# gregversteeg/LinearCorex

Hardware: NVIDIA B200
Metric: fit_iters_per_sec (higher is better)
Workload: dtype f64 (6 int8 digit planes = 48 bits, exact int32 products, f64 recombination)

## Files before the change

### linearcorex_b200/csrc/host_gram.cuh

```cuda
#pragma once
#include "host_oz.cuh"

static long long gram_tbuf_doubles(const lcx_session* s, int block_cols) {
    return ((long long)s->L.S * block_cols * s->L.ldk8 + 7) / 8;
}

static long long gram_scratch_doubles(const lcx_session* s, int block_cols, long long ldg) {
    return round_up(block_cols, 16) + align16(gram_tbuf_doubles(s, block_cols)) +
           (s->L.oz_build_splits > 1 ? (long long)s->L.oz_build_splits * block_cols * ldg : 0LL) + 64;
}

template <int S>
static int gram_build_t(lcx_session* s, double* g, long long ldg, int B, double* scratch) {
    const Layout& L = s->L;
    const int n = s->n;
    double* scale = scratch;
    int8_t* tbuf = (int8_t*)(scratch + round_up(B, 16));
    double* part = scratch + round_up(B, 16) + align16(gram_tbuf_doubles(s, B));
    const long long t_stride = (long long)B * L.ldk8;
    const int splits = L.oz_build_splits;
    oz::gram_scale_kernel<<<cdiv(B, 256), 256, 0, s->stream>>>(s->oz_xscale(), 1.0 / (double)s->Nt, scale, B);
    LAUNCHED(s);
    for (int c0 = 0; c0 < n; c0 += B) {
        const int nb = min(B, n - c0);
        oz::transpose_planes_kernel<<<dim3((unsigned)cdiv(s->Nl, 128), cdiv(nb, 128), S), dim3(32, 8), 0, s->stream>>>(
            s->xs(), L.ld8, s->Nl, s->Nl * L.ld8, c0, nb, tbuf, L.ldk8, t_stride);
        LAUNCHED(s);
        const int bnm = oz::bn_max(S);
        const int n_tiles = cdiv(nb, bnm);
        const int bn = (int)max(16LL, round_up(cdiv(nb, n_tiles), bnm > 64 ? 16 : 8));
        CUtensorMap map_a, map_b;
        LCX_TRY(oz::make_slice_map(&map_a, s->xs() + c0, n - c0, s->Nl, S, L.ld8, s->Nl * L.ld8, oz::kBM, oz::kBK, true));
        LCX_TRY(oz::make_slice_map(&map_b, tbuf, s->Nl, nb, S, L.ldk8, t_stride, oz::kBK, bn, false));
        oz::GemmParams p;
        memset(&p, 0, sizeof(p));
        double* dst = g + (long long)c0 * ldg + c0;
        p.C = splits > 1 ? part : dst;
        p.ldc = ldg;
        p.c_split_stride = splits > 1 ? (long long)B * ldg : 0;
        p.col_scale = scale;
        p.inv_radix = 1.0 / (double)L.radix;
        p.rows = n - c0; p.cols = nb; p.k_total = (int)s->Nl; p.k_chunk = L.oz_build_chunk;
        p.bn = bn;
        p.trans_out = 1;
        LCX_TRY((oz::launch_oz_gemm<S, false>(map_a, map_b, p, dim3(n_tiles, cdiv(n - c0, oz::kBM), splits), s->stream, oz_cluster())));
        LAUNCHED(s);
        if (splits > 1) {
            LCX_TRY(launch_reduce_splits(part, splits, (long long)B * ldg, dst, nb, n - c0, ldg, s->stream));
            LAUNCHED(s);
        }
    }
    oz::mirror_upper_kernel<<<dim3(cdiv(n, 32), cdiv(n, 32)), dim3(32, 8), 0, s->stream>>>(g, ldg, n);
    LAUNCHED(s);
    LCX_CUDA(cudaGetLastError());
    return 0;
}

static int gram_build(lcx_session* s, double* g, long long ldg, int B, double* scratch) {
    switch (s->L.S) {
        case 3: return gram_build_t<3>(s, g, ldg, B, scratch);
        case 4: return gram_build_t<4>(s, g, ldg, B, scratch);
        case 5: return gram_build_t<5>(s, g, ldg, B, scratch);
        case 6: return gram_build_t<6>(s, g, ldg, B, scratch);
        case 7: return gram_build_t<7>(s, g, ldg, B, scratch);
    }
    return fail(LCX_ERR_STATE, "gram_build", "bad digit count");
}

template <int S>
static int gram_pair_t(lcx_session* s, const double* A, double* svec, cudaEvent_t* ev, const double* dot_b, double* dot_out,
                       bool leave_partials) {
    const Layout& L = s->L;
    const int m = s->m, n = s->n;
    double* D = s->ptr(LCX_A_D);
    if (s->row_parts > 0 && dot_out != nullptr) {
        oz::slice_rows_part_kernel<S><<<dim3(m, cdiv(L.ld8, 4 * 128)), 128, 0, s->stream>>>(
            A, L.ld, m, n, s->ptr(I_FROW), s->ptr(I_FROW) + (long long)kSMs * L.ldm, s->row_parts, L.ldm, s->oz_xscale(),
            s->oz_ascale(), s->oz_cscale(), dot_out, s->as(), L.ld8, (long long)m * L.ld8, (double)L.radix);
        LAUNCHED(s);
    } else {
    oz::row_scale_kernel<<<m, 256, 0, s->stream>>>(A, L.ld, n, s->oz_ascale(), 0, s->oz_xscale(), s->oz_cscale(), dot_b, dot_out);
    LAUNCHED(s);
    oz::slice_rows_kernel<S><<<dim3(m, cdiv(L.ld8, 4 * 128)), 128, 0, s->stream>>>(A, L.ld, m, n, s->oz_ascale(), nullptr, s->as(), L.ld8,
                                                                              (long long)m * L.ld8, (double)L.radix);
    LAUNCHED(s);
    }
    oz::GemmParams p;
    memset(&p, 0, sizeof(p));
    p.ldc = L.ld;
    p.col_scale = s->oz_cscale();
    p.inv_radix = 1.0 / (double)L.radix;
    p.rows = n; p.cols = m; p.k_total = n;
    p.bn = s->oz_bn;
    p.trans_out = 1;
    s->d_splits = 1;
    const int n_tiles = cdiv(m, oz::bn_max(S));
    if (s->peers.world > 1) {
        const int P = s->peers.world, m_tiles = cdiv(n, oz::kBM);
        const int per = cdiv(m_tiles, P);
        const int t0 = min(m_tiles, s->peers.rank * per), t1 = min(m_tiles, t0 + per);
        const int mine = t1 - t0;
        const int clusters = kSMs / 2, kblocks = cdiv(n, oz::kBK);
        const long long col0 = (long long)t0 * oz::kBM;
        const int ncols = (int)(min((long long)L.ld, (long long)t1 * oz::kBM) - col0);
        if (mine > 0) {
            const int smin = cdiv(n, L.oz_kmax), smax = max(smin, min(clusters, max(1, kblocks / 4)));
            int sp = smin;
            double best = 1e300;
            for (int c = smin; c <= smax; ++c) {
                const int rounds = cdiv((long long)mine * c, clusters);
                const double cost = rounds * (ceil((double)kblocks / c) + oz_unit_fixed_kb()) + (c > 1 ? 1.5 * c : 0.0);
                if (cost < best - 1e-9) { best = cost; sp = c; }
            }
            const int chunk = (int)round_up(cdiv(n, sp), oz::kBK);
            const int splits = cdiv(n, chunk);
            LCX_REQUIRE((long long)splits * m * L.ld <= L.slot[I_PART][0].cols, "split-K partial buffer too small");
// ... 93 lines not shown
```

### linearcorex_b200/csrc/host_oz.cuh

```cuda
#pragma once
#include "host_session.cuh"

template <int S>
static int oz_slice_x_t(lcx_session* s) {
    const Layout& L = s->L;
    oz::absmax_partial_kernel<<<kAmaxCtas, 256, 0, s->stream>>>(s->xt, s->ldx, s->Nl, s->n, s->ws + L.slot[I_AMAX][0].off);
    LAUNCHED(s);
    oz::absmax_finish_kernel<<<1, 256, 0, s->stream>>>(s->ws + L.slot[I_AMAX][0].off, kAmaxCtas, s->oz_xscale());
    LAUNCHED(s);
    dim3 grid((unsigned)s->Nl, cdiv(L.ld8, 4 * 128));
    oz::slice_rows_kernel<S><<<grid, 128, 0, s->stream>>>(s->xt, s->ldx, (int)s->Nl, s->n, nullptr, s->oz_xscale(), s->xs(), L.ld8,
                                                        s->Nl * L.ld8, (double)L.radix);
    LAUNCHED(s);
    LCX_CUDA(cudaGetLastError());
    return 0;
}

static int oz_prepare(lcx_session* s, bool streamed) {
    const Layout& L = s->L;
    LCX_REQUIRE(L.oz1_chunk <= L.oz_kmax && L.oz_chunk <= L.oz_kmax, "contraction chunk exceeds the int32-exact length");
    if (!streamed) switch (L.S) {
        case 3: LCX_TRY(oz_slice_x_t<3>(s)); break;
        case 4: LCX_TRY(oz_slice_x_t<4>(s)); break;
        case 5: LCX_TRY(oz_slice_x_t<5>(s)); break;
        case 6: LCX_TRY(oz_slice_x_t<6>(s)); break;
        case 7: LCX_TRY(oz_slice_x_t<7>(s)); break;
        default: return fail(LCX_ERR_STATE, "oz_prepare", "bad digit count");
    }
    LCX_TRY(oz::make_slice_map(&s->map_x_k1, s->xs(), s->n, s->Nl, L.S, L.ld8, s->Nl * L.ld8, oz::kBK, oz::kBM, false));
    const int bnm = oz::bn_max(L.S);
    const int n_tiles = cdiv(s->m, bnm);
    s->oz_bn = (int)max(16LL, round_up(cdiv(s->m, n_tiles), bnm > 64 ? 16 : 8));
    const int bn = s->oz_bn;
    LCX_TRY(oz::make_slice_map(&s->map_a_k1, s->as(), s->n, s->m, L.S, L.ld8, (long long)s->m * L.ld8, oz::kBK, bn, false));
    LCX_TRY(oz::make_slice_map(&s->map_x_k2, s->xs(), s->n, s->Nl, L.S, L.ld8, s->Nl * L.ld8, oz::kBM, oz::kBK, true));
    LCX_TRY(oz::make_slice_map(&s->map_y_k2, s->ys(), s->Nl, s->m, L.S, L.ldk8, (long long)s->m * L.ldk8, oz::kBK, bn, false));
    if (L.mm_i8) {
        LCX_REQUIRE(L.mm_chunk <= L.oz_kmax && round_up(s->m, oz::kBK) <= L.oz_kmax, "contraction chunk exceeds the int32-exact length");
        const long long st_n = (long long)s->m * L.ld8, st_q = (long long)s->m * L.ldm8;
        LCX_TRY(oz::make_slice_map(&s->map_mm_a, s->mma(), s->n, s->m, L.S, L.ld8, st_n, oz::kBK, oz::kBM, false));
        LCX_TRY(oz::make_slice_map(&s->map_mm_b, s->mmb(), s->n, s->m, L.S, L.ld8, st_n, oz::kBK, bn, false));
        LCX_TRY(oz::make_slice_map(&s->map_mn_c, s->mmc(), s->n, s->m, L.S, L.ld8, st_n, oz::kBM, oz::kBK, true));
        LCX_TRY(oz::make_slice_map(&s->map_mn_q, s->mmq(), s->m, s->m, L.S, L.ldm8, st_q, oz::kBK, bn, false));
    }
    return 0;
}

static int oz_cluster() {
    const char* env = getenv("LCX_OZ_CLUSTER");
    return env ? atoi(env) : 2;
}

template <int S>
static int oz_pair_t(lcx_session* s, const double* A, double* svec, cudaEvent_t* ev, bool first_only, bool want_tail,
                     const double* dot_b, double* dot_out) {
    const Layout& L = s->L;
    const int m = s->m, n = s->n;
    double* Y = s->ptr(LCX_A_Y);
    double* D = s->ptr(LCX_A_D);
    if (s->row_parts > 0 && dot_out != nullptr) {
        oz::slice_rows_part_kernel<S><<<dim3(m, cdiv(L.ld8, 4 * 128)), 128, 0, s->stream>>>(
            A, L.ld, m, n, s->ptr(I_FROW), s->ptr(I_FROW) + (long long)kSMs * L.ldm, s->row_parts, L.ldm, s->oz_xscale(),
            s->oz_ascale(), s->oz_cscale(), dot_out, s->as(), L.ld8, (long long)m * L.ld8, (double)L.radix);
        LAUNCHED(s);
    } else {
    oz::row_scale_kernel<<<m, 256, 0, s->stream>>>(A, L.ld, n, s->oz_ascale(), 0, s->oz_xscale(), s->oz_cscale(), dot_b, dot_out);
    LAUNCHED(s);
    oz::slice_rows_kernel<S><<<dim3(m, cdiv(L.ld8, 4 * 128)), 128, 0, s->stream>>>(A, L.ld, m, n, s->oz_ascale(), nullptr, s->as(), L.ld8,
                                                                              (long long)m * L.ld8, (double)L.radix);
    LAUNCHED(s);
    }
    {
        oz::GemmParams p;
        memset(&p, 0, sizeof(p));
        const bool split1 = L.oz1_splits > 1;
        p.C = split1 ? s->ptr(I_PART) : Y;
        p.ldc = L.ldy; p.c_split_stride = split1 ? s->Nl * L.ldy : 0;
        p.col_scale = s->oz_cscale();
        p.inv_radix = 1.0 / (double)L.radix;
        p.rows = (int)s->Nl; p.cols = m; p.k_total = n; p.k_chunk = L.oz1_chunk;
        p.bn = s->oz_bn;
        const int row0 = (cdiv(s->Nl, oz::kBM) - L.oz1_tail_tiles) * oz::kBM;
        if (L.oz1_tail_tiles > 0) {
            const int groups = cdiv(cdiv(m, oz::bn_max(S)), 2), m_tiles = cdiv(s->Nl, oz::kBM);
            p.main_units = groups * (m_tiles * L.oz1_splits - L.oz1_tail_tiles);
            p.tail_units = groups * L.oz1_tail_tiles * L.oz1_tail_splits;
            p.tail_m_tile0 = m_tiles - L.oz1_tail_tiles; p.tail_m_tiles = L.oz1_tail_tiles;
            p.tail_kbase = (L.oz1_splits - 1) * L.oz1_chunk; p.tail_kchunk = L.oz1_tail_chunk;
            p.tail_C = s->ptr(I_TAIL1) - (long long)row0 * L.ldy;
            p.tail_ldc = L.ldy; p.tail_split_stride = (long long)L.oz1_tail_tiles * oz::kBM * L.ldy;
        }
        LCX_TRY((oz::launch_oz_gemm<S, true>(s->map_x_k1, s->map_a_k1, p,
                                             dim3(cdiv(m, oz::bn_max(S)), cdiv(s->Nl, oz::kBM), L.oz1_splits), s->stream, oz_cluster())));
        LAUNCHED(s);
        if (L.oz1_tail_tiles > 0) {
            double* dst = (split1 ? s->ptr(I_PART) + (long long)(L.oz1_splits - 1) * s->Nl * L.ldy : Y) + (long long)row0 * L.ldy;
            const int rows = (int)(s->Nl - row0);
            oz::tail_fold_kernel<<<cdiv((long long)rows * m, 256), 256, 0, s->stream>>>(
                s->ptr(I_TAIL1), L.oz1_tail_splits, (long long)L.oz1_tail_tiles * oz::kBM * L.ldy, L.ldy, dst, L.ldy, rows, m);
            LAUNCHED(s);
        }
        if (split1) {
            LCX_TRY(launch_reduce_splits(s->ptr(I_PART), L.oz1_splits, s->Nl * L.ldy, Y, (int)s->Nl, m, L.ldy, s->stream));
            LAUNCHED(s);
        }
    }
    if (ev) LCX_CUDA(cudaEventRecord(ev[1], s->stream));
    if (ev) LCX_CUDA(cudaEventRecord(ev[3], s->stream));
    double* ystat = s->ws + L.slot[I_YSTAT][0].off;
    oz::y_stats_kernel<<<dim3(cdiv(m, 32), L.ystat_slabs), dim3(32, 8), 0, s->stream>>>(Y, L.ldy, s->Nl, m, kYStatRows, ystat, L.ldm);
    LAUNCHED(s);
    oz::y_stats_finish_kernel<<<m, 256, 0, s->stream>>>(ystat, L.ystat_slabs, L.ldm, m, s->oz_xscale(), svec, s->oz_yscale(),
                                                                  s->oz_dscale());
    LAUNCHED(s);
    if (first_only) {
        LCX_CUDA(cudaGetLastError());
        return 0;
    }
    oz::slice_cols_t_kernel<S><<<dim3((unsigned)cdiv(s->Nl, 128), cdiv(m, 32)), dim3(32, 8), 0, s->stream>>>(
        Y, L.ldy, s->Nl, m, s->oz_yscale(), s->ys(), L.ldk8, (long long)m * L.ldk8, (double)L.radix);
    LAUNCHED(s);
    {
        oz::GemmParams p;
        memset(&p, 0, sizeof(p));
        const bool split = L.oz_splits > 1;
        p.C = split ? s->ptr(I_PART) : D;
// ... 156 lines not shown
```

### linearcorex_b200/csrc/ozaki_i8.cuh

```cuda
#pragma once
#include <cuda.h>

#include "common.cuh"

namespace lcx {
namespace oz {

constexpr int kBM = 128;
constexpr int kBK = 64;
__host__ __device__ constexpr int bn_max(int S) { return S <= 4 ? 128 : 64; }
__host__ __device__ constexpr int stages_for(int S) {
    return (220 * 1024) / (S * (kBM * kBK + bn_max(S) * kBK)) >= 4 ? 4 : (220 * 1024) / (S * (kBM * kBK + bn_max(S) * kBK));
}
constexpr int kThreads = 192;

__device__ __forceinline__ void mbar_init(uint64_t* bar, uint32_t count) {
    asm volatile("mbarrier.init.shared::cta.b64 [%0], %1;" ::"r"(smem_u32(bar)), "r"(count));
}
__device__ __forceinline__ void mbar_expect_tx(uint64_t* bar, uint32_t bytes) {
    asm volatile("mbarrier.arrive.expect_tx.shared::cta.b64 _, [%0], %1;" ::"r"(smem_u32(bar)), "r"(bytes) : "memory");
}
__device__ __forceinline__ void mbar_arrive(uint64_t* bar) {
    asm volatile("mbarrier.arrive.shared::cta.b64 _, [%0];" ::"r"(smem_u32(bar)) : "memory");
}
__device__ __forceinline__ void mbar_wait(uint64_t* bar, uint32_t parity) {
    asm volatile(
        "{\n\t"
        ".reg .pred p;\n\t"
        "WAIT_LOOP:\n\t"
        "mbarrier.try_wait.parity.shared::cta.b64 p, [%0], %1;\n\t"
        "@p bra DONE;\n\t"
        "bra WAIT_LOOP;\n\t"
        "DONE:\n\t"
        "}\n" ::"r"(smem_u32(bar)),
        "r"(parity)
        : "memory");
}
__device__ __forceinline__ void tma_load_3d(void* dst, const CUtensorMap* map, uint64_t* bar, int c0, int c1, int c2) {
    asm volatile(
        "cp.async.bulk.tensor.3d.shared::cluster.global.mbarrier::complete_tx::bytes [%0], [%1, {%3, %4, %5}], [%2];" ::"r"(
            smem_u32(dst)),
        "l"(map), "r"(smem_u32(bar)), "r"(c0), "r"(c1), "r"(c2)
        : "memory");
}
__device__ __forceinline__ void tma_load_3d_mc(void* dst, const CUtensorMap* map, uint64_t* bar, int c0, int c1, int c2,
                                               uint16_t mask) {
    asm volatile(
        "cp.async.bulk.tensor.3d.shared::cluster.global.mbarrier::complete_tx::bytes.multicast::cluster [%0], [%1, {%4, %5, %6}], "
        "[%2], %3;" ::"r"(smem_u32(dst)),
        "l"(map), "r"(smem_u32(bar)), "h"(mask), "r"(c0), "r"(c1), "r"(c2)
        : "memory");
}
__device__ __forceinline__ void umma_commit_mc(uint64_t* bar, uint16_t mask) {
    asm volatile("tcgen05.commit.cta_group::1.mbarrier::arrive::one.shared::cluster.multicast::cluster.b64 [%0], %1;" ::"r"(
                     smem_u32(bar)),
                 "h"(mask)
                 : "memory");
}
__device__ __forceinline__ bool elect_one_sync() {
    uint32_t pred;
    asm volatile(
        "{\n\t"
        ".reg .pred p;\n\t"
        "elect.sync _|p, 0xffffffff;\n\t"
        "selp.b32 %0, 1, 0, p;\n\t"
        "}\n"
        : "=r"(pred));
    return pred != 0;
}
__device__ __forceinline__ uint32_t cluster_ctarank() {
    uint32_t r;
    asm volatile("mov.u32 %0, %%cluster_ctarank;" : "=r"(r));
    return r;
}
__device__ __forceinline__ void cluster_sync_all() {
    asm volatile("barrier.cluster.arrive.release.aligned;" ::: "memory");
    asm volatile("barrier.cluster.wait.acquire.aligned;" ::: "memory");
}
__device__ __forceinline__ void tmem_alloc(uint32_t* dst_smem, uint32_t cols) {
    asm volatile("tcgen05.alloc.cta_group::1.sync.aligned.shared::cta.b32 [%0], %1;" ::"r"(smem_u32(dst_smem)), "r"(cols));
    asm volatile("tcgen05.relinquish_alloc_permit.cta_group::1.sync.aligned;");
}
__device__ __forceinline__ void tmem_dealloc(uint32_t taddr, uint32_t cols) {
    asm volatile("tcgen05.dealloc.cta_group::1.sync.aligned.b32 %0, %1;" ::"r"(taddr), "r"(cols));
}
__device__ __forceinline__ void umma_i8(uint32_t d_tmem, uint64_t a_desc, uint64_t b_desc, uint32_t idesc, uint32_t accumulate) {
    asm volatile(
        "{\n\t"
        ".reg .pred p;\n\t"
        "setp.ne.b32 p, %4, 0;\n\t"
        "tcgen05.mma.cta_group::1.kind::i8 [%0], %1, %2, %3, p;\n\t"
        "}\n" ::"r"(d_tmem),
        "l"(a_desc), "l"(b_desc), "r"(idesc), "r"(accumulate));
}
__device__ __forceinline__ void umma_commit(uint64_t* bar) {
    asm volatile("tcgen05.commit.cta_group::1.mbarrier::arrive::one.shared::cluster.b64 [%0];" ::"r"(smem_u32(bar)) : "memory");
}
__device__ __forceinline__ void tmem_ld16(uint32_t taddr, uint32_t (&r)[16]) {
    asm volatile(
        "tcgen05.ld.sync.aligned.32x32b.x16.b32 {%0,%1,%2,%3,%4,%5,%6,%7,%8,%9,%10,%11,%12,%13,%14,%15}, [%16];"
        : "=r"(r[0]), "=r"(r[1]), "=r"(r[2]), "=r"(r[3]), "=r"(r[4]), "=r"(r[5]), "=r"(r[6]), "=r"(r[7]), "=r"(r[8]), "=r"(r[9]),
          "=r"(r[10]), "=r"(r[11]), "=r"(r[12]), "=r"(r[13]), "=r"(r[14]), "=r"(r[15])
        : "r"(taddr));
}
__device__ __forceinline__ void tmem_ld_wait() { asm volatile("tcgen05.wait::ld.sync.aligned;" ::: "memory"); }
__device__ __forceinline__ void tc_fence_before() { asm volatile("tcgen05.fence::before_thread_sync;" ::: "memory"); }
__device__ __forceinline__ void tc_fence_after() { asm volatile("tcgen05.fence::after_thread_sync;" ::: "memory"); }

__device__ __forceinline__ uint64_t make_smem_desc(uint32_t saddr, uint32_t lbo_bytes, uint32_t sbo_bytes, uint32_t layout) {
    uint64_t d = 0;
    d |= (uint64_t)((saddr >> 4) & 0x3FFF);
    d |= (uint64_t)((lbo_bytes >> 4) & 0x3FFF) << 16;
    d |= (uint64_t)((sbo_bytes >> 4) & 0x3FFF) << 32;
    d |= (uint64_t)1 << 46;
    d |= (uint64_t)(layout & 7) << 61;
    return d;
}

__host__ __device__ constexpr uint32_t make_idesc_i8(int M, int N, int a_mn, int b_mn) {
    return (2u << 4) | (1u << 7) | (1u << 10) | ((uint32_t)a_mn << 15) | ((uint32_t)b_mn << 16) | ((uint32_t)(N >> 3) << 17) |
           ((uint32_t)(M >> 4) << 24);
}

struct GemmParams {
    double* C;
    long long ldc;
    long long c_split_stride;
    const double* row_scale;
    const double* col_scale;
    int rows, cols;
    int k_total;
    int k_chunk;
    double inv_radix;
    int n_tiles;
    int n_groups, m_tiles, k_splits;
    int n_tile0;
    int m_tile0;
    int bn;
    int trans_out;
    int debug;
    const double* c_add;
    int main_units;
    int tail_units;
    int tail_m_tile0, tail_m_tiles;
    int tail_kbase, tail_kchunk;
    double* tail_C;
    long long tail_ldc, tail_split_stride;
};

template <int S, bool KMAJOR, int BN>
__device__ __forceinline__ void issue_kblock(uint32_t sa, uint32_t sb, uint32_t tmem_base, bool first_block) {
    constexpr int A_BYTES = kBM * kBK;
    constexpr int B_BYTES = BN * kBK;
    constexpr bool ODD8 = (BN % 16) != 0;
    constexpr int CMAX = ODD8 ? ((256 / BN) & ~1) : (256 / BN);
    static_assert(BN % 8 == 0 && BN >= 16 && CMAX >= 1, "tile width");
#pragma unroll
    for (int kk = 0; kk < kBK / 32; ++kk) {
#pragma unroll
        for (int ka = 0; ka < S; ++ka) {
            constexpr int kMaxInstr = S;
            int q0 = 0;
#pragma unroll
            for (int it = 0; it < kMaxInstr; ++it) {
                const int left = S - ka - q0;
                if (left <= 0) break;
                int cnt = left < CMAX ? left : CMAX;
                int n = BN * cnt;
                if (ODD8) {
                    if (cnt >= 2) { cnt &= ~1; n = BN * cnt; }
                    else n = BN + 8;
                }
                const uint32_t idesc = make_idesc_i8(kBM, n, KMAJOR ? 0 : 1, 0);
                const uint64_t da = KMAJOR ? make_smem_desc(sa + ka * A_BYTES + kk * 32, 16, 512, 4)
                                           : make_smem_desc(sa + ka * A_BYTES + kk * 4096, 8192, 1024, 2);
                const uint64_t db = make_smem_desc(sb + q0 * B_BYTES + kk * 32, 16, 512, 4);
                const uint32_t acc = (!first_block || kk > 0 || ka > 0) ? 1u : 0u;
                umma_i8(tmem_base + (uint32_t)((ka + q0) * BN), da, db, idesc, acc);
                q0 += cnt;
            }
        }
    }
}

template <int S, bool KMAJOR, int CL, bool CADD = false>
__global__ void __launch_bounds__(kThreads, 1)
oz_gemm_kernel(const __grid_constant__ CUtensorMap mapA, const __grid_constant__ CUtensorMap mapB, const GemmParams p) {
    constexpr int kBN = bn_max(S);
    constexpr int kStages = stages_for(S);
    constexpr int A_BYTES = kBM * kBK;
    constexpr int B_BYTES = kBN * kBK;
    constexpr int STAGE_BYTES = S * (A_BYTES + B_BYTES);
    constexpr uint32_t TMEM_COLS = (S * kBN + 8 <= 128) ? 128 : (S * kBN + 8 <= 256 ? 256 : 512);
    static_assert(S * kBN <= 512, "accumulators exceed TMEM");
    static_assert(kStages >= 2, "pipeline needs two stages");

    extern __shared__ __align__(1024) uint8_t smem_raw[];
    uint8_t* smem = (uint8_t*)(((uintptr_t)smem_raw + 1023) & ~(uintptr_t)1023);
    __shared__ __align__(8) uint64_t full_bar[kStages];
    __shared__ __align__(8) uint64_t empty_bar[kStages];
    __shared__ __align__(8) uint64_t tmem_full_bar;
    __shared__ __align__(8) uint64_t tmem_empty_bar;
    __shared__ uint32_t tmem_base_smem;

    const int warp = threadIdx.x >> 5, lane = threadIdx.x & 31;
    const uint32_t crank = (CL > 1) ? cluster_ctarank() : 0u;
    constexpr uint16_t kMask = (uint16_t)((1u << CL) - 1u);
    const int bn = p.bn;
    const int b_bytes = bn * kBK;
    const int cluster_id = (int)blockIdx.x / CL, n_clusters = (int)gridDim.x / CL;
    const int units_main = p.main_units > 0 ? p.main_units : p.n_groups * p.m_tiles * p.k_splits;
    const int units = units_main + p.tail_units;

    if (warp == 0 && lane == 0) {
        asm volatile("prefetch.tensormap [%0];" ::"l"(&mapA) : "memory");
        asm volatile("prefetch.tensormap [%0];" ::"l"(&mapB) : "memory");
        for (int i = 0; i < kStages; ++i) {
            mbar_init(&full_bar[i], 1);
            mbar_init(&empty_bar[i], CL);
        }
        mbar_init(&tmem_full_bar, 1);
        mbar_init(&tmem_empty_bar, 4);
        asm volatile("fence.mbarrier_init.release.cluster;" ::: "memory");
    }
    if (warp == 1) tmem_alloc(&tmem_base_smem, TMEM_COLS);
    tc_fence_before();
    __syncthreads();
    if (CL > 1) cluster_sync_all();
    tc_fence_after();
    const uint32_t tmem_base = tmem_base_smem;

    auto unit_of = [&](int u, int& n_tile, int& m_tile, int& z, int& kbeg, int& num_kb) {
        int kend;
        if (u < units_main) {
            const int g = u % p.n_groups;
            const int r = u / p.n_groups;
            m_tile = p.m_tile0 + r % p.m_tiles;
            z = r / p.m_tiles;
            n_tile = p.n_tile0 + g * CL + (int)crank;
            kbeg = z * p.k_chunk;
            kend = min(p.k_total, kbeg + p.k_chunk);
        } else {
            const int v = u - units_main;
            const int g = v % p.n_groups;
            const int r = v / p.n_groups;
            m_tile = p.tail_m_tile0 + r % p.tail_m_tiles;
            const int zt = r / p.tail_m_tiles;
            z = -1 - zt;
            n_tile = p.n_tile0 + g * CL + (int)crank;
            kbeg = p.tail_kbase + zt * p.tail_kchunk;
            kend = min(p.k_total, kbeg + p.tail_kchunk);
        }
        num_kb = (kend > kbeg) ? (kend - kbeg + kBK - 1) / kBK : 0;
    };

    if (warp == 0) {
        {
            uint32_t kbg = 0;
            for (int u = cluster_id; u < units; u += n_clusters) {
                int n_tile, m_tile, z, kbeg, num_kb;
                unit_of(u, n_tile, m_tile, z, kbeg, num_kb);
                for (int kb = 0; kb < num_kb; ++kb, ++kbg) {
                    const uint32_t st = kbg % kStages;
                    const uint32_t ph = (kbg / kStages) & 1;
                    mbar_wait(&empty_bar[st], ph ^ 1);
                    uint8_t* sa = smem + st * STAGE_BYTES;
                    uint8_t* sb = sa + S * A_BYTES;
                    const bool load_a = !(p.debug & 2), load_b = !(p.debug & 4);
                    const int k0 = kbeg + kb * kBK;
                    if (elect_one_sync()) {
                        mbar_expect_tx(&full_bar[st], S * ((load_a ? A_BYTES : 0) + (load_b ? b_bytes : 0)));
#pragma unroll
                        for (int s = 0; s < S; ++s) {
                            if (!load_a) {
                            } else if (CL == 1) {
                                if (KMAJOR) tma_load_3d(sa + s * A_BYTES, &mapA, &full_bar[st], k0, m_tile * kBM, s);
                                else tma_load_3d(sa + s * A_BYTES, &mapA, &full_bar[st], m_tile * kBM, k0, s);
                            } else if ((uint32_t)(s % CL) == crank) {
                                if (KMAJOR) tma_load_3d_mc(sa + s * A_BYTES, &mapA, &full_bar[st], k0, m_tile * kBM, s, kMask);
                                else tma_load_3d_mc(sa + s * A_BYTES, &mapA, &full_bar[st], m_tile * kBM, k0, s, kMask);
                            }
                            if (load_b) tma_load_3d(sb + s * b_bytes, &mapB, &full_bar[st], k0, n_tile * bn, s);
                        }
                    }
                    __syncwarp();
                }
            }
        }
    } else if (warp == 1) {
        {
            uint32_t kbg = 0, it = 0;
            for (int u = cluster_id; u < units; u += n_clusters) {
                int n_tile, m_tile, z, kbeg, num_kb;
                unit_of(u, n_tile, m_tile, z, kbeg, num_kb);
                if (num_kb == 0) continue;
                if (it > 0) {
                    mbar_wait(&tmem_empty_bar, (it - 1) & 1);
                    tc_fence_after();
                }
                ++it;
                for (int kb = 0; kb < num_kb; ++kb, ++kbg) {
                    const uint32_t st = kbg % kStages;
                    const uint32_t ph = (kbg / kStages) & 1;
                    mbar_wait(&full_bar[st], ph);
                    tc_fence_after();
                    const uint32_t sa = smem_u32(smem + st * STAGE_BYTES);
                    const uint32_t sb = sa + S * A_BYTES;
                    if (elect_one_sync()) {
                    bool wide = (p.debug & 1) != 0;
                    if constexpr (kBN > 64) {
                        wide = wide || bn > 64;
                        if (p.debug & 1) {
                        } else if (bn == 128) issue_kblock<S, KMAJOR, 128>(sa, sb, tmem_base, kb == 0);
                        else if (bn == 112) issue_kblock<S, KMAJOR, 112>(sa, sb, tmem_base, kb == 0);
                        else if (bn == 96) issue_kblock<S, KMAJOR, 96>(sa, sb, tmem_base, kb == 0);
                        else if (bn == 80) issue_kblock<S, KMAJOR, 80>(sa, sb, tmem_base, kb == 0);
                    }
                    if (wide) {
                    } else if (bn == 64) issue_kblock<S, KMAJOR, 64>(sa, sb, tmem_base, kb == 0);
                    else if (bn == 56) issue_kblock<S, KMAJOR, 56>(sa, sb, tmem_base, kb == 0);
                    else if (bn == 48) issue_kblock<S, KMAJOR, 48>(sa, sb, tmem_base, kb == 0);
                    else if (bn == 40) issue_kblock<S, KMAJOR, 40>(sa, sb, tmem_base, kb == 0);
                    else if (bn == 32) issue_kblock<S, KMAJOR, 32>(sa, sb, tmem_base, kb == 0);
                    else if (bn == 24) issue_kblock<S, KMAJOR, 24>(sa, sb, tmem_base, kb == 0);
                    else issue_kblock<S, KMAJOR, 16>(sa, sb, tmem_base, kb == 0);
                    if (CL == 1) umma_commit(&empty_bar[st]);
                    else umma_commit_mc(&empty_bar[st], kMask);
                    }
                    __syncwarp();
                }
                if (elect_one_sync()) umma_commit(&tmem_full_bar);
                __syncwarp();
            }
        }
    } else {
        const int quarter = warp & 3;
        const int row_in_tile = quarter * 32 + lane;
        const uint32_t lane_addr = tmem_base + ((uint32_t)(quarter * 32) << 16);
        uint32_t it = 0;
        for (int u = cluster_id; u < units; u += n_clusters) {
            int n_tile, m_tile, z, kbeg, num_kb;
            unit_of(u, n_tile, m_tile, z, kbeg, num_kb);
            const int row = m_tile * kBM + row_in_tile;
            double cadd[16];
            auto fetch_cadd = [&](int c0) {
#pragma unroll
                for (int j = 0; j < 16; ++j) {
                    const int col = n_tile * bn + c0 + j;
                    cadd[j] = (row < p.rows && col < p.cols && c0 + j < bn) ? p.c_add[(long long)col * p.ldc + row] : 0.0;
                }
            };
            if (CADD) fetch_cadd(0);
// ... 392 lines not shown
    }
    mx = block_max_256(mx, scratch);
    if (threadIdx.x == 0) part[blockIdx.x] = mx;
}
__global__ void absmax_finish_kernel(const double* __restrict__ part, int nparts, double* __restrict__ scale) {
    __shared__ double scratch[8];
    double mx = 0.0;
    for (int i = threadIdx.x; i < nparts; i += 256) mx = fmax(mx, part[i]);
    mx = block_max_256(mx, scratch);
    if (threadIdx.x == 0) scale[0] = pow2_above(mx);
}

__global__ void __launch_bounds__(256) transpose_planes_kernel(const int8_t* __restrict__ in, long long ld_in, long long rows,
                                                               long long in_slice_stride, int c0, int ncols,
                                                               int8_t* __restrict__ out, long long ld_out,
                                                               long long out_slice_stride) {
    constexpr int PITCH = 132;
    __shared__ __align__(4) int8_t t[128][PITCH];
    const int tx = threadIdx.x, ty = threadIdx.y;
    const long long r0 = (long long)blockIdx.x * 128;
    const int cb = blockIdx.y * 128;
    const int8_t* src = in + (long long)blockIdx.z * in_slice_stride;
    int8_t* dst = out + (long long)blockIdx.z * out_slice_stride;
#pragma unroll 4
    for (int i = 0; i < 16; ++i) {
        const int rr = ty + 8 * i;
        const long long r = r0 + rr;
        uint32_t w = 0;
        if (r < rows && c0 + cb + 4 * tx < ld_in) w = *reinterpret_cast<const uint32_t*>(src + r * ld_in + c0 + cb + 4 * tx);
        t[4 * tx + 0][rr] = (int8_t)(w & 0xff);
        t[4 * tx + 1][rr] = (int8_t)((w >> 8) & 0xff);
        t[4 * tx + 2][rr] = (int8_t)((w >> 16) & 0xff);
        t[4 * tx + 3][rr] = (int8_t)((w >> 24) & 0xff);
    }
    __syncthreads();
    if (r0 + 4 * tx >= ld_out) return;
    for (int c = ty; c < 128; c += 8) {
        if (cb + c < ncols)
            *reinterpret_cast<uint32_t*>(dst + (long long)(cb + c) * ld_out + r0 + 4 * tx) =
                *reinterpret_cast<const uint32_t*>(&t[c][4 * tx]);
    }
}

__global__ void gram_scale_kernel(const double* __restrict__ x_scale, double factor, double* __restrict__ out, int count) {
    const int i = blockIdx.x * blockDim.x + threadIdx.x;
    if (i < count) out[i] = x_scale[0] * x_scale[0] * factor;
}

__global__ void __launch_bounds__(256) mirror_upper_kernel(double* __restrict__ g, long long ld, int n) {
    __shared__ double t[32][33];
    const int ti = blockIdx.y, tj = blockIdx.x;
    if (ti < tj) return;
    const int tx = threadIdx.x, ty = threadIdx.y;
#pragma unroll
    for (int k = 0; k < 4; ++k) {
        const int r = tj * 32 + ty + 8 * k, c = ti * 32 + tx;
        t[ty + 8 * k][tx] = (r < n && c < n) ? g[(long long)r * ld + c] : 0.0;
    }
    __syncthreads();
#pragma unroll
    for (int k = 0; k < 4; ++k) {
        const int r = ti * 32 + ty + 8 * k, c = tj * 32 + tx;
        if (r < n && c < n && r > c) g[(long long)r * ld + c] = t[tx][ty + 8 * k];
    }
}

typedef CUresult (*EncodeTiledFn)(CUtensorMap*, CUtensorMapDataType, cuuint32_t, void*, const cuuint64_t*, const cuuint64_t*,
                                  const cuuint32_t*, const cuuint32_t*, CUtensorMapInterleave, CUtensorMapSwizzle,
                                  CUtensorMapL2promotion, CUtensorMapFloatOOBfill);

inline EncodeTiledFn encode_fn() {
    static EncodeTiledFn fn = nullptr;
    if (fn == nullptr) {
        void* p = nullptr;
        cudaDriverEntryPointQueryResult q;
        if (cudaGetDriverEntryPoint("cuTensorMapEncodeTiled", &p, cudaEnableDefault, &q) == cudaSuccess &&
            q == cudaDriverEntryPointSuccess)
            fn = (EncodeTiledFn)p;
    }
    return fn;
}

inline int make_slice_map(CUtensorMap* map, const void* base, long long inner, long long rows, int slices, long long ld,
                          long long slice_stride, int box_inner, int box_rows, bool swizzle128) {
    EncodeTiledFn fn = encode_fn();
    if (!fn) return fail(-2, "cuTensorMapEncodeTiled", "driver entry point unavailable");
    cuuint64_t dims[3] = {(cuuint64_t)inner, (cuuint64_t)rows, (cuuint64_t)slices};
    cuuint64_t strides[2] = {(cuuint64_t)ld, (cuuint64_t)slice_stride};
    cuuint32_t box[3] = {(cuuint32_t)box_inner, (cuuint32_t)box_rows, 1};
    cuuint32_t estr[3] = {1, 1, 1};
    CUtensorMapL2promotion promo = CU_TENSOR_MAP_L2_PROMOTION_L2_256B;
    if (const char* env = getenv("LCX_OZ_L2PROMO")) {
        const int v = atoi(env);
        promo = v == 0 ? CU_TENSOR_MAP_L2_PROMOTION_NONE : v == 64 ? CU_TENSOR_MAP_L2_PROMOTION_L2_64B
              : v == 128 ? CU_TENSOR_MAP_L2_PROMOTION_L2_128B : CU_TENSOR_MAP_L2_PROMOTION_L2_256B;
    }
    CUresult rc = fn(map, CU_TENSOR_MAP_DATA_TYPE_UINT8, 3, const_cast<void*>(base), dims, strides, box, estr,
                     CU_TENSOR_MAP_INTERLEAVE_NONE, swizzle128 ? CU_TENSOR_MAP_SWIZZLE_128B : CU_TENSOR_MAP_SWIZZLE_64B, promo,
                     CU_TENSOR_MAP_FLOAT_OOB_FILL_NONE);
    if (rc != CUDA_SUCCESS) return fail(-2, "cuTensorMapEncodeTiled", "encode failed (check alignment / strides)");
    return 0;
}

inline bool oz_persistent() {
    static int v = -1;
    if (v < 0) {
        const char* env = getenv("LCX_OZ_PERSISTENT");
        v = (env && atoi(env) == 0) ? 0 : 1;
    }
    return v != 0;
}

template <int S, bool KMAJOR, int CL, bool CADD = false>
inline int launch_oz_gemm_cl(const CUtensorMap& mapA, const CUtensorMap& mapB, GemmParams p, dim3 grid, cudaStream_t st) {
    constexpr int SMEM = stages_for(S) * S * (kBM * kBK + bn_max(S) * kBK) + 1024;
    static PerDeviceOnce configured = {};
    static int resident[64] = {};
    auto kern = oz_gemm_kernel<S, KMAJOR, CL, CADD>;
    if (configured.first_time()) LCX_CUDA(cudaFuncSetAttribute(kern, cudaFuncAttributeMaxDynamicSharedMemorySize, SMEM));
    p.n_groups = (int)round_up(grid.x, CL) / CL;
    p.m_tiles = (int)grid.y;
    p.k_splits = (int)grid.z;
    const long long units = (p.main_units > 0 ? (long long)p.main_units : (long long)p.n_groups * p.m_tiles * p.k_splits) + p.tail_units;
    {
        static int dbg = -1;
        if (dbg < 0) {
            const char* env = getenv("LCX_OZ_DEBUG");
            dbg = env ? atoi(env) : 0;
        }
        p.debug = dbg;
    }
    cudaLaunchConfig_t cfg;
    memset(&cfg, 0, sizeof(cfg));
    cfg.blockDim = dim3(kThreads);
    cfg.dynamicSmemBytes = SMEM;
    cfg.stream = st;
    cudaLaunchAttribute attr[1];
    attr[0].id = cudaLaunchAttributeClusterDimension;
    attr[0].val.clusterDim.x = CL;
    attr[0].val.clusterDim.y = 1;
    attr[0].val.clusterDim.z = 1;
    cfg.attrs = attr;
    cfg.numAttrs = 1;
    int dev = 0;
    LCX_CUDA(cudaGetDevice(&dev));
    dev &= 63;
    if (resident[dev] == 0) {
        int n = 0, sms = 0;
        cfg.gridDim = dim3(CL * 1024);
        if (cudaOccupancyMaxActiveClusters(&n, kern, &cfg) != cudaSuccess || n <= 0) {
            cudaGetLastError();
            LCX_CUDA(cudaDeviceGetAttribute(&sms, cudaDevAttrMultiProcessorCount, dev));
            n = sms / CL;
        }
        resident[dev] = n > 0 ? n : 1;
    }
    const long long clusters = oz_persistent() ? (units < resident[dev] ? units : resident[dev]) : units;
    LCX_REQUIRE(clusters * CL < (1LL << 31), "grid too large");
    cfg.gridDim = dim3((unsigned)(clusters * CL));
    LCX_CUDA(cudaLaunchKernelEx(&cfg, kern, mapA, mapB, p));
    return 0;
}

template <int S, bool KMAJOR, bool CADD = false>
inline int launch_oz_gemm(const CUtensorMap& mapA, const CUtensorMap& mapB, GemmParams p, dim3 grid, cudaStream_t st,
                          int cluster) {
    const int n_tiles = (int)grid.x;
    p.n_tiles = n_tiles;
    p.n_tile0 = 0;
    if (CADD) cluster = cluster > 2 ? 2 : cluster;
    if (!CADD && cluster >= 4 && n_tiles >= 4) return launch_oz_gemm_cl<S, KMAJOR, 4, false>(mapA, mapB, p, grid, st);
    if (cluster >= 2 && n_tiles >= 2) {
        if (n_tiles % 2 == 0) return launch_oz_gemm_cl<S, KMAJOR, 2, CADD>(mapA, mapB, p, grid, st);
        if (n_tiles > 3) {
            grid.x = (unsigned)(n_tiles - 3);
            const int rc = launch_oz_gemm_cl<S, KMAJOR, 2, CADD>(mapA, mapB, p, grid, st);
            if (rc != 0) return rc;
        }
        p.n_tile0 = n_tiles - 3;
        grid.x = 3;
        return launch_oz_gemm_cl<S, KMAJOR, 3, CADD>(mapA, mapB, p, grid, st);
    }
    return launch_oz_gemm_cl<S, KMAJOR, 1, CADD>(mapA, mapB, p, grid, st);
}

}
}
```

Baseline: 240.1.

## Halve GEMM stage depth to 32 bytes, double pipeline stages, add optional TMA prefetch

Shrinks each pipeline stage's K extent from 64 to 32 int8 elements, so each stage holds one UMMA K step. The stage count rises from 4 to up to 8, and tensor maps switch to 32B swizzle for the K-major operands, with the shared-memory descriptors changed to match. This aims for finer-grained, deeper producer/consumer overlap. It also adds an env-gated L2 prefetch of upcoming tiles, off by default. The cost is twice as many mbarrier round trips and smaller TMA transactions, plus a risk of worse bank behaviour with the narrower swizzle.

```diff
diff --git a/linearcorex_b200/csrc/host_gram.cuh b/linearcorex_b200/csrc/host_gram.cuh
--- a/linearcorex_b200/csrc/host_gram.cuh
+++ b/linearcorex_b200/csrc/host_gram.cuh
@@ -30,8 +30,8 @@
         const int n_tiles = cdiv(nb, bnm);
         const int bn = (int)max(16LL, round_up(cdiv(nb, n_tiles), bnm > 64 ? 16 : 8));
         CUtensorMap map_a, map_b;
-        LCX_TRY(oz::make_slice_map(&map_a, s->xs() + c0, n - c0, s->Nl, S, L.ld8, s->Nl * L.ld8, oz::kBM, oz::kBK, true));
-        LCX_TRY(oz::make_slice_map(&map_b, tbuf, s->Nl, nb, S, L.ldk8, t_stride, oz::kBK, bn, false));
+        LCX_TRY(oz::make_slice_map(&map_a, s->xs() + c0, n - c0, s->Nl, S, L.ld8, s->Nl * L.ld8, oz::kBM, oz::kSK));
+        LCX_TRY(oz::make_slice_map(&map_b, tbuf, s->Nl, nb, S, L.ldk8, t_stride, oz::kSK, bn));
         oz::GemmParams p;
         memset(&p, 0, sizeof(p));
         double* dst = g + (long long)c0 * ldg + c0;
diff --git a/linearcorex_b200/csrc/host_oz.cuh b/linearcorex_b200/csrc/host_oz.cuh
--- a/linearcorex_b200/csrc/host_oz.cuh
+++ b/linearcorex_b200/csrc/host_oz.cuh
@@ -27,21 +27,21 @@
         case 7: LCX_TRY(oz_slice_x_t<7>(s)); break;
         default: return fail(LCX_ERR_STATE, "oz_prepare", "bad digit count");
     }
-    LCX_TRY(oz::make_slice_map(&s->map_x_k1, s->xs(), s->n, s->Nl, L.S, L.ld8, s->Nl * L.ld8, oz::kBK, oz::kBM, false));
+    LCX_TRY(oz::make_slice_map(&s->map_x_k1, s->xs(), s->n, s->Nl, L.S, L.ld8, s->Nl * L.ld8, oz::kSK, oz::kBM));
     const int bnm = oz::bn_max(L.S);
     const int n_tiles = cdiv(s->m, bnm);
     s->oz_bn = (int)max(16LL, round_up(cdiv(s->m, n_tiles), bnm > 64 ? 16 : 8));
     const int bn = s->oz_bn;
-    LCX_TRY(oz::make_slice_map(&s->map_a_k1, s->as(), s->n, s->m, L.S, L.ld8, (long long)s->m * L.ld8, oz::kBK, bn, false));
-    LCX_TRY(oz::make_slice_map(&s->map_x_k2, s->xs(), s->n, s->Nl, L.S, L.ld8, s->Nl * L.ld8, oz::kBM, oz::kBK, true));
-    LCX_TRY(oz::make_slice_map(&s->map_y_k2, s->ys(), s->Nl, s->m, L.S, L.ldk8, (long long)s->m * L.ldk8, oz::kBK, bn, false));
+    LCX_TRY(oz::make_slice_map(&s->map_a_k1, s->as(), s->n, s->m, L.S, L.ld8, (long long)s->m * L.ld8, oz::kSK, bn));
+    LCX_TRY(oz::make_slice_map(&s->map_x_k2, s->xs(), s->n, s->Nl, L.S, L.ld8, s->Nl * L.ld8, oz::kBM, oz::kSK));
+    LCX_TRY(oz::make_slice_map(&s->map_y_k2, s->ys(), s->Nl, s->m, L.S, L.ldk8, (long long)s->m * L.ldk8, oz::kSK, bn));
     if (L.mm_i8) {
         LCX_REQUIRE(L.mm_chunk <= L.oz_kmax && round_up(s->m, oz::kBK) <= L.oz_kmax, "contraction chunk exceeds the int32-exact length");
         const long long st_n = (long long)s->m * L.ld8, st_q = (long long)s->m * L.ldm8;
-        LCX_TRY(oz::make_slice_map(&s->map_mm_a, s->mma(), s->n, s->m, L.S, L.ld8, st_n, oz::kBK, oz::kBM, false));
-        LCX_TRY(oz::make_slice_map(&s->map_mm_b, s->mmb(), s->n, s->m, L.S, L.ld8, st_n, oz::kBK, bn, false));
-        LCX_TRY(oz::make_slice_map(&s->map_mn_c, s->mmc(), s->n, s->m, L.S, L.ld8, st_n, oz::kBM, oz::kBK, true));
-        LCX_TRY(oz::make_slice_map(&s->map_mn_q, s->mmq(), s->m, s->m, L.S, L.ldm8, st_q, oz::kBK, bn, false));
+        LCX_TRY(oz::make_slice_map(&s->map_mm_a, s->mma(), s->n, s->m, L.S, L.ld8, st_n, oz::kSK, oz::kBM));
+        LCX_TRY(oz::make_slice_map(&s->map_mm_b, s->mmb(), s->n, s->m, L.S, L.ld8, st_n, oz::kSK, bn));
+        LCX_TRY(oz::make_slice_map(&s->map_mn_c, s->mmc(), s->n, s->m, L.S, L.ld8, st_n, oz::kBM, oz::kSK));
+        LCX_TRY(oz::make_slice_map(&s->map_mn_q, s->mmq(), s->m, s->m, L.S, L.ldm8, st_q, oz::kSK, bn));
     }
     return 0;
 }
diff --git a/linearcorex_b200/csrc/ozaki_i8.cuh b/linearcorex_b200/csrc/ozaki_i8.cuh
--- a/linearcorex_b200/csrc/ozaki_i8.cuh
+++ b/linearcorex_b200/csrc/ozaki_i8.cuh
@@ -8,10 +8,10 @@
 
 constexpr int kBM = 128;
 constexpr int kBK = 64;
+constexpr int kSK = 32;
 __host__ __device__ constexpr int bn_max(int S) { return S <= 4 ? 128 : 64; }
-__host__ __device__ constexpr int stages_for(int S) {
-    return (220 * 1024) / (S * (kBM * kBK + bn_max(S) * kBK)) >= 4 ? 4 : (220 * 1024) / (S * (kBM * kBK + bn_max(S) * kBK));
-}
+__host__ __device__ constexpr int stage_bytes(int S) { return S * (kBM * kSK + bn_max(S) * kSK); }
+__host__ __device__ constexpr int stages_for(int S) { return (220 * 1024) / stage_bytes(S) >= 8 ? 8 : (220 * 1024) / stage_bytes(S); }
 constexpr int kThreads = 192;
 
 __device__ __forceinline__ void mbar_init(uint64_t* bar, uint32_t count) {
@@ -50,6 +50,10 @@
         "[%2], %3;" ::"r"(smem_u32(dst)),
         "l"(map), "r"(smem_u32(bar)), "h"(mask), "r"(c0), "r"(c1), "r"(c2)
         : "memory");
+}
+__device__ __forceinline__ void tma_prefetch_3d(const CUtensorMap* map, int c0, int c1, int c2) {
+    asm volatile("cp.async.bulk.prefetch.tensor.3d.L2.global.tile [%0, {%1, %2, %3}];" ::"l"(map), "r"(c0), "r"(c1), "r"(c2)
+                 : "memory");
 }
 __device__ __forceinline__ void umma_commit_mc(uint64_t* bar, uint16_t mask) {
     asm volatile("tcgen05.commit.cta_group::1.mbarrier::arrive::one.shared::cluster.multicast::cluster.b64 [%0], %1;" ::"r"(
@@ -139,6 +143,8 @@
     int bn;
     int trans_out;
     int debug;
+    int prefetch;
+    int prefetch_b;
     const double* c_add;
     int main_units;
     int tail_units;
@@ -150,13 +156,13 @@
 
 template <int S, bool KMAJOR, int BN>
 __device__ __forceinline__ void issue_kblock(uint32_t sa, uint32_t sb, uint32_t tmem_base, bool first_block) {
-    constexpr int A_BYTES = kBM * kBK;
-    constexpr int B_BYTES = BN * kBK;
+    constexpr int A_BYTES = kBM * kSK;
+    constexpr int B_BYTES = BN * kSK;
     constexpr bool ODD8 = (BN % 16) != 0;
     constexpr int CMAX = ODD8 ? ((256 / BN) & ~1) : (256 / BN);
     static_assert(BN % 8 == 0 && BN >= 16 && CMAX >= 1, "tile width");
-#pragma unroll
-    for (int kk = 0; kk < kBK / 32; ++kk) {
+    static_assert(kSK == 32, "one UMMA K step per stage");
+    {
 #pragma unroll
         for (int ka = 0; ka < S; ++ka) {
             constexpr int kMaxInstr = S;
@@ -172,10 +178,10 @@
                     else n = BN + 8;
                 }
                 const uint32_t idesc = make_idesc_i8(kBM, n, KMAJOR ? 0 : 1, 0);
-                const uint64_t da = KMAJOR ? make_smem_desc(sa + ka * A_BYTES + kk * 32, 16, 512, 4)
-                                           : make_smem_desc(sa + ka * A_BYTES + kk * 4096, 8192, 1024, 2);
-                const uint64_t db = make_smem_desc(sb + q0 * B_BYTES + kk * 32, 16, 512, 4);
-                const uint32_t acc = (!first_block || kk > 0 || ka > 0) ? 1u : 0u;
+                const uint64_t da = KMAJOR ? make_smem_desc(sa + ka * A_BYTES, 16, 256, 6)
+                                           : make_smem_desc(sa + ka * A_BYTES, 8192, 1024, 2);
+                const uint64_t db = make_smem_desc(sb + q0 * B_BYTES, 16, 256, 6);
+                const uint32_t acc = (!first_block || ka > 0) ? 1u : 0u;
                 umma_i8(tmem_base + (uint32_t)((ka + q0) * BN), da, db, idesc, acc);
                 q0 += cnt;
             }
@@ -188,9 +194,9 @@
 oz_gemm_kernel(const __grid_constant__ CUtensorMap mapA, const __grid_constant__ CUtensorMap mapB, const GemmParams p) {
     constexpr int kBN = bn_max(S);
     constexpr int kStages = stages_for(S);
-    constexpr int A_BYTES = kBM * kBK;
-    constexpr int B_BYTES = kBN * kBK;
-    constexpr int STAGE_BYTES = S * (A_BYTES + B_BYTES);
+    constexpr int A_BYTES = kBM * kSK;
+    constexpr int B_BYTES = kBN * kSK;
+    constexpr int STAGE_BYTES = stage_bytes(S);
     constexpr uint32_t TMEM_COLS = (S * kBN + 8 <= 128) ? 128 : (S * kBN + 8 <= 256 ? 256 : 512);
     static_assert(S * kBN <= 512, "accumulators exceed TMEM");
     static_assert(kStages >= 2, "pipeline needs two stages");
@@ -207,7 +213,7 @@
     const uint32_t crank = (CL > 1) ? cluster_ctarank() : 0u;
     constexpr uint16_t kMask = (uint16_t)((1u << CL) - 1u);
     const int bn = p.bn;
-    const int b_bytes = bn * kBK;
+    const int b_bytes = bn * kSK;
     const int cluster_id = (int)blockIdx.x / CL, n_clusters = (int)gridDim.x / CL;
     const int units_main = p.main_units > 0 ? p.main_units : p.n_groups * p.m_tiles * p.k_splits;
     const int units = units_main + p.tail_units;
@@ -251,23 +257,48 @@
             kbeg = p.tail_kbase + zt * p.tail_kchunk;
             kend = min(p.k_total, kbeg + p.tail_kchunk);
         }
-        num_kb = (kend > kbeg) ? (kend - kbeg + kBK - 1) / kBK : 0;
+        num_kb = (kend > kbeg) ? (kend - kbeg + kSK - 1) / kSK : 0;
     };
 
     if (warp == 0) {
         {
+            const bool load_a = !(p.debug & 2), load_b = !(p.debug & 4);
+            int pu = cluster_id - n_clusters, pkb = 0, pnum = 0, pn_tile = 0, pm_tile = 0, pkbeg = 0;
+            auto prefetch_next = [&]() {
+                while (pkb >= pnum) {
+                    pu += n_clusters;
+                    if (pu >= units) return;
+                    int pz;
+                    unit_of(pu, pn_tile, pm_tile, pz, pkbeg, pnum);
+                    pkb = 0;
+                }
+                const int k0 = pkbeg + pkb * kSK;
+                if (elect_one_sync()) {
+#pragma unroll
+                    for (int s = 0; s < S; ++s) {
+                        if (load_a && (uint32_t)(s % CL) == crank) {
+                            if (KMAJOR) tma_prefetch_3d(&mapA, k0, pm_tile * kBM, s);
+                            else tma_prefetch_3d(&mapA, pm_tile * kBM, k0, s);
+                        }
+                        if (load_b && p.prefetch_b) tma_prefetch_3d(&mapB, k0, pn_tile * bn, s);
+                    }
+                }
+                __syncwarp();
+                ++pkb;
+            };
+            for (int i = 0; i < p.prefetch; ++i) prefetch_next();
             uint32_t kbg = 0;
             for (int u = cluster_id; u < units; u += n_clusters) {
                 int n_tile, m_tile, z, kbeg, num_kb;
                 unit_of(u, n_tile, m_tile, z, kbeg, num_kb);
                 for (int kb = 0; kb < num_kb; ++kb, ++kbg) {
+                    if (p.prefetch > 0) prefetch_next();
                     const uint32_t st = kbg % kStages;
                     const uint32_t ph = (kbg / kStages) & 1;
                     mbar_wait(&empty_bar[st], ph ^ 1);
                     uint8_t* sa = smem + st * STAGE_BYTES;
                     uint8_t* sb = sa + S * A_BYTES;
-                    const bool load_a = !(p.debug & 2), load_b = !(p.debug & 4);
-                    const int k0 = kbeg + kb * kBK;
+                    const int k0 = kbeg + kb * kSK;
                     if (elect_one_sync()) {
                         mbar_expect_tx(&full_bar[st], S * ((load_a ? A_BYTES : 0) + (load_b ? b_bytes : 0)));
 #pragma unroll
@@ -826,7 +857,8 @@
 }
 
 inline int make_slice_map(CUtensorMap* map, const void* base, long long inner, long long rows, int slices, long long ld,
-                          long long slice_stride, int box_inner, int box_rows, bool swizzle128) {
+                          long long slice_stride, int box_inner, int box_rows) {
+    if (box_inner != 32 && box_inner != 128) return fail(-2, "make_slice_map", "box inner extent must be 32 or 128 bytes");
     EncodeTiledFn fn = encode_fn();
     if (!fn) return fail(-2, "cuTensorMapEncodeTiled", "driver entry point unavailable");
     cuuint64_t dims[3] = {(cuuint64_t)inner, (cuuint64_t)rows, (cuuint64_t)slices};
@@ -840,7 +872,7 @@
               : v == 128 ? CU_TENSOR_MAP_L2_PROMOTION_L2_128B : CU_TENSOR_MAP_L2_PROMOTION_L2_256B;
     }
     CUresult rc = fn(map, CU_TENSOR_MAP_DATA_TYPE_UINT8, 3, const_cast<void*>(base), dims, strides, box, estr,
-                     CU_TENSOR_MAP_INTERLEAVE_NONE, swizzle128 ? CU_TENSOR_MAP_SWIZZLE_128B : CU_TENSOR_MAP_SWIZZLE_64B, promo,
+                     CU_TENSOR_MAP_INTERLEAVE_NONE, box_inner == 128 ? CU_TENSOR_MAP_SWIZZLE_128B : CU_TENSOR_MAP_SWIZZLE_32B, promo,
                      CU_TENSOR_MAP_FLOAT_OOB_FILL_NONE);
     if (rc != CUDA_SUCCESS) return fail(-2, "cuTensorMapEncodeTiled", "encode failed (check alignment / strides)");
     return 0;
@@ -855,9 +887,19 @@
     return v != 0;
 }
 
+inline int oz_prefetch_kb() {
+    const char* env = getenv("LCX_OZ_PREFETCH");
+    const int v = env ? atoi(env) : 0;
+    return v > 0 ? v : 0;
+}
+inline int oz_prefetch_b() {
+    const char* env = getenv("LCX_OZ_PREFETCH_B");
+    return (env && atoi(env) != 0) ? 1 : 0;
+}
+
 template <int S, bool KMAJOR, int CL, bool CADD = false>
 inline int launch_oz_gemm_cl(const CUtensorMap& mapA, const CUtensorMap& mapB, GemmParams p, dim3 grid, cudaStream_t st) {
-    constexpr int SMEM = stages_for(S) * S * (kBM * kBK + bn_max(S) * kBK) + 1024;
+    constexpr int SMEM = stages_for(S) * stage_bytes(S) + 1024;
     static PerDeviceOnce configured = {};
     static int resident[64] = {};
     auto kern = oz_gemm_kernel<S, KMAJOR, CL, CADD>;
@@ -874,6 +916,8 @@
         }
         p.debug = dbg;
     }
+    p.prefetch = oz_prefetch_kb();
+    p.prefetch_b = oz_prefetch_b();
     cudaLaunchConfig_t cfg;
     memset(&cfg, 0, sizeof(cfg));
     cfg.blockDim = dim3(kThreads);
```

Result: slower. 213.4 (median of 6 runs) (-11.1%).
